# CloudEngineHub/MARL-LLM

Measured on AMD Instinct MI355X. Metric: agent-steps/sec, higher is better.
Workload: dtype f64 (state, every index / flag / reward decision) + f32 (obs, prior, action I/O, pre-filters); 1 GPU; assembly env, 64 agents x 4096 envs per GPU (64 x 4096 total), assembled state, prior-policy actions; agents=64, envs_per_gpu=4096, envs_total=4096, obs_dtype=f32, state_dtype=f64, seed=226, parallelism=env-sharded x1, no collective on the step path

## Files before the change

### marl_llm_amd/csrc/swarm_env.hip

```cpp

#include <hip/hip_runtime.h>

#include <algorithm>
#include <cmath>
#include <cstdint>
#include <cstdio>
#include <cstring>
#include <mutex>
#include <new>
#include <string>
#include <type_traits>
#include <utility>
#include <vector>

#include "swarm_env.h"
#include "swarm_internal.h"

namespace {

constexpr int kTopoMax = 6;
constexpr int kNeiStride = 8;
typedef unsigned long long u64;

struct LatEnv {
    double ox, oy;
    double uxi, uyi, vxi, vyi;
    float R, Rc;
    int nrows, ncols;
    short rowstart[64];
    unsigned long long rowmask[64];
};

struct KP {
    int n_env, n_a, ng_max, ngw, topo, g_max, occ_max, obs_dim;
    int with_self, periodic, boundary, with_prior, export_idx;
    int export_small;
    int cxy_stride;
    int cxq_stride;
    int g_stride;
    int off_cxy, off_sp, off_cmask, off_sbits, off_obits, off_sidx, off_snei, off_sncf, off_snear, off_pc;
    int smem_lat, smem_lat_export, smem_generic;
    double c_sen, c_near, c_occ, c_avoid, c_ball;
    double c_close, c_close2;
    float csen_lo, csen_hi, cocc_lo, cocc_hi;
    float coord_lim;
    float min_tol_a, min_tol_b;
    float rew_ga, rew_gb;
    int force_exact;
    int cap_int;
    unsigned cap_magic; int cap_shift;
    int cap_even;
    int dbg_phase, dbg_extra;
    int off_cxyf, off_partc, off_lat, off_cov, off_flag;
    int off_hdr, off_srow, off_pcr, off_perm, off_rres, off_orow, off_partd;
    float rew_ga_lat, rew_gb_lat;
    float rew_thr_k;
    int lattice;
    int lat_rw, lat_cw;
    int lat_nrs, lat_nrc;
    int lat_n32;
    double c_near_hi;
    const LatEnv *lat;
    double d_sen, r_avoid, size_a, size2, k_ball, k_wall, c_wall, vel_max, dt;
    double bx0, by1, bx2, by3, w_half, h_half;
    double *p, *dp;
    int *nei, *near_cell, *in_flag;
    double2 *sf_next;
    const double *cells;
    const double2 *cells_xy;
    const int *n_g;
    const double *c_in;
    int *exp_sensed, *exp_occ;
    void *prior_next;
    double pk_att, pk_rep, pk_ali;
    double pk_llm;
    int llm;
    double2 *act_next;
    long long *stamps;
};

typedef float f2v __attribute__((ext_vector_type(2)));

template <typename T> struct Pair;
template <> struct Pair<float>  { typedef float2 type; };
template <> struct Pair<double> { typedef double2 type; };
typedef __attribute__((ext_vector_type(2))) __bf16 bf2v;
template <> struct Pair<__bf16> { typedef bf2v type; };

template <typename OT> __device__ __forceinline__ OT to_out(double v) { return (OT)v; }
typedef double d2v __attribute__((ext_vector_type(2)));
__device__ __forceinline__ void store_nt(float2 *dst, float2 v) { f2v t = {v.x, v.y}; __builtin_nontemporal_store(t, reinterpret_cast<f2v *>(dst)); }
__device__ __forceinline__ void store_nt(double2 *dst, double2 v) { d2v t = {v.x, v.y}; __builtin_nontemporal_store(t, reinterpret_cast<d2v *>(dst)); }
__device__ __forceinline__ void store_nt(bf2v *dst, bf2v v) { __builtin_nontemporal_store(v, dst); }
template <> __device__ __forceinline__ __bf16 to_out<__bf16>(double v) { return (__bf16)(float)v; }

__device__ __forceinline__ void wrap_rel(double &x, double &y, double wh, double hh)
{
    if (x < -wh) x += 2 * wh; else if (x > wh) x -= 2 * wh;
    if (y < -hh) y += 2 * hh; else if (y > hh) y -= 2 * hh;
}


template <int LANE>
__device__ __forceinline__ int writelane_c(int value, int old)
{
    asm("s_nop 1\n\tv_writelane_b32 %0, %1, %2" : "+v"(old) : "s"(value), "n"(LANE));
    return old;
}

__device__ __forceinline__ unsigned shl1_or_mask(unsigned acc, unsigned long long mask)
{
    unsigned long long carry_out;
    asm("s_nop 1\n\tv_addc_co_u32_e64 %0, %1, %2, %2, %3" : "=v"(acc), "=s"(carry_out) : "v"(acc), "s"(mask));
    return acc;
}

__device__ __forceinline__ void pair_tests5(double d2u, double d2, double c_nb, double c_hi, double c_ht, double c_cd, double c_c1,
                                            unsigned &nb, unsigned &hi, unsigned &ht, unsigned &cd, unsigned &c1)
{
    unsigned long long m0, m1, m2, m3, m4;
    asm("v_cmp_lt_f64_e64 %5, %10, %12\n\t"
        "v_cmp_lt_f64_e64 %6, %10, %13\n\t"
        "v_cmp_lt_f64_e64 %7, %10, %14\n\t"
        "v_cmp_lt_f64_e64 %8, %11, %15\n\t"
        "v_cmp_lt_f64_e64 %9, %11, %16\n\t"
        "v_addc_co_u32_e64 %0, %5, %0, %0, %5\n\t"
        "v_addc_co_u32_e64 %1, %6, %1, %1, %6\n\t"
        "v_addc_co_u32_e64 %2, %7, %2, %2, %7\n\t"
        "v_addc_co_u32_e64 %3, %8, %3, %3, %8\n\t"
        "v_addc_co_u32_e64 %4, %9, %4, %4, %9"
        : "+v"(nb), "+v"(hi), "+v"(ht), "+v"(cd), "+v"(c1), "=&s"(m0), "=&s"(m1), "=&s"(m2), "=&s"(m3), "=&s"(m4)
        : "v"(d2u), "v"(d2), "s"(c_nb), "s"(c_hi), "s"(c_ht), "s"(c_cd), "s"(c_c1));
}

__device__ __forceinline__ void pair_tests6(double d2u, double d2, double c_nb, double c_hi, double c_ht, double c_cd, double c_c1, double c_c2,
                                            unsigned &nb, unsigned &hi, unsigned &ht, unsigned &cd, unsigned &c1, unsigned &c2)
{
    unsigned long long m0, m1, m2, m3, m4, m5;
    asm("v_cmp_lt_f64_e64 %6, %12, %14\n\t"
        "v_cmp_lt_f64_e64 %7, %12, %15\n\t"
        "v_cmp_lt_f64_e64 %8, %12, %16\n\t"
        "v_cmp_lt_f64_e64 %9, %13, %17\n\t"
        "v_cmp_lt_f64_e64 %10, %13, %18\n\t"
        "v_cmp_lt_f64_e64 %11, %13, %19\n\t"
        "v_addc_co_u32_e64 %0, %6, %0, %0, %6\n\t"
        "v_addc_co_u32_e64 %1, %7, %1, %1, %7\n\t"
        "v_addc_co_u32_e64 %2, %8, %2, %2, %8\n\t"
        "v_addc_co_u32_e64 %3, %9, %3, %3, %9\n\t"
        "v_addc_co_u32_e64 %4, %10, %4, %4, %10\n\t"
        "v_addc_co_u32_e64 %5, %11, %5, %5, %11"
        : "+v"(nb), "+v"(hi), "+v"(ht), "+v"(cd), "+v"(c1), "+v"(c2), "=&s"(m0), "=&s"(m1), "=&s"(m2), "=&s"(m3), "=&s"(m4), "=&s"(m5)
        : "v"(d2u), "v"(d2), "s"(c_nb), "s"(c_hi), "s"(c_ht), "s"(c_cd), "s"(c_c1), "s"(c_c2));
}

template <typename F, int... I>
__device__ __forceinline__ void static_for_impl(F &&f, std::integer_sequence<int, I...>)
{
    (f(std::integral_constant<int, I>{}), ...);
}
template <int N, typename F>
__device__ __forceinline__ void static_for(F &&f)
{
    static_for_impl(static_cast<F &&>(f), std::make_integer_sequence<int, N>{});
}

__device__ __forceinline__ double clamp_ref(double v, double lo, double hi)
{
    double m = (hi < v) ? hi : v;
    return (lo < m) ? m : lo;
}

#define REPS(k) ((P.dbg_phase == (k)) ? P.dbg_extra + 1 : 1)
#define FENCE() asm volatile("" ::: "memory")
#define EXIT_AT(k) do { if (P.dbg_phase == 15 && P.dbg_extra == (k)) return; } while (0)

#ifdef SWARM_STAMPS
#define STAMP(k) do { __builtin_amdgcn_sched_barrier(0); if (P.stamps != nullptr && (threadIdx.x & 63) == 0) P.stamps[((size_t)blockIdx.x * (blockDim.x >> 6) + (threadIdx.x >> 6)) * 24 + (k)] = clock64(); __builtin_amdgcn_sched_barrier(0); } while (0)
#else
#define STAMP(k) do { } while (0)
#endif

template <int NPAD, bool HALF = false> struct Geo {
    static_assert(!HALF || NPAD < 64, "the half-occupied geometry is for N < 64");
    static constexpr int NPAD_ = NPAD; static constexpr bool HALF_ = HALF;
    static constexpr bool CT_MAP = NPAD >= 64 || HALF;
    static constexpr int AG = NPAD < 64 ? 64 : NPAD;
    static constexpr int EPB = NPAD < 64 ? (64 / NPAD) / (HALF ? 2 : 1) : 1;
    static constexpr int ACTW = NPAD < 64 ? EPB * NPAD : 64;
    static constexpr int LPA = HALF ? 8 : 4;
    static constexpr int AGW = 64 / LPA;
    static constexpr int NW = AG / 64;
    static constexpr int WPE = 4;
    static constexpr int T = AG * WPE;
#ifndef SWARM_WPS
#define SWARM_WPS 7
#endif
#ifndef SWARM_WPS_SMALL
#define SWARM_WPS_SMALL 6
#endif
#ifndef SWARM_WPS_128
#define SWARM_WPS_128 6
#endif
    static constexpr int WPS_LAT = NPAD == 64 ? SWARM_WPS : (NPAD < 64 ? SWARM_WPS_SMALL : (NPAD == 128 ? SWARM_WPS_128 : 1));
    static constexpr int WPS_GEN = NPAD == 64 ? 6 : (NPAD < 64 ? 5 : 1);
};

template <int NPAD, bool HALF> struct LatMap {
    typedef Geo<NPAD, HALF> G_;
    static constexpr int AG = G_::AG, EPB = G_::EPB, NW = G_::NW, WPE = G_::WPE, T = G_::T;
    static constexpr int NRC = 16;
    static constexpr int al(int bytes) { return (bytes + 15) & ~15; }
    static constexpr int mx(int a, int b) { return a > b ? a : b; }
    static constexpr int sp_bytes = 4 * AG * 8;
    static constexpr int hdr_bytes = AG * 16;
    static constexpr int rew_scratch_bytes = NW * 1536;
    static constexpr int srow_bytes = mx((NRC - 1) * AG * 4, rew_scratch_bytes);
    static constexpr int pcr_bytes = AG * NRC;
    static constexpr int partc_bytes = WPE * AG * 2;
    static constexpr int partd_bytes = (WPE - 1) * AG * 8;
    static constexpr int lat_bytes = EPB * 64 * (8 + 2);
    static constexpr int cov_bytes = EPB * 64 * 8;
    static constexpr int flag_bytes = AG;
    static constexpr int snei_bytes = AG * kNeiStride * 2;
    static constexpr int sncf_bytes = AG * 4;
    static constexpr int snear_bytes = NW > 1 ? NW * AG * 8 : 0;
    static constexpr int orow_bytes = NRC * AG * 4;
    static constexpr int pm_bytes = (NW == 1 ? WPE * 4 : 5) * NW * AG * 8;
    static constexpr int sp = 0;
    static constexpr int hdr = sp + al(sp_bytes);
    static constexpr int srow = hdr + al(hdr_bytes);
    static constexpr int pcr = srow + al(srow_bytes);
    static constexpr int partc = pcr + al(pcr_bytes);
    static constexpr int partd = partc + al(partc_bytes);
    static constexpr int lat = partd + al(partd_bytes);
    static constexpr int cov = lat + al(lat_bytes);
    static constexpr int flag = cov + al(cov_bytes);
    static constexpr int snei = flag + al(flag_bytes);
    static constexpr int sncf = snei + al(snei_bytes);
    static constexpr int snear = sncf + al(sncf_bytes);
    static constexpr int sidx = snear + al(snear_bytes);
    static constexpr int perm = partd;
    static constexpr int perm_bytes = T, prk_bytes = WPE * AG * 2;
    static constexpr int sidx_bytes(int g_stride) { return al(mx(AG * g_stride * 2, pm_bytes)); }
    static constexpr int total(int g_stride) { return sidx + sidx_bytes(g_stride); }
    static constexpr int orow_off(int g_stride) { return total(g_stride); }
    static constexpr int total_export(int g_stride) { return orow_off(g_stride) + al(orow_bytes); }
    static_assert(perm_bytes <= partd_bytes, "perm must fit the distance array it reuses");
    static_assert(prk_bytes <= partc_bytes, "the partial ranks must fit the nearest-cell candidates they reuse");
    static_assert(rew_scratch_bytes <= srow_bytes, "the exact reward's scratch must fit the window rows it reuses");
    static_assert(pm_bytes <= sidx_bytes(0), "the pair masks must fit the list region they reuse");
};

constexpr double kSentinel = 1.0e200;

__device__ __forceinline__ double cospi01(double t)
{
    const bool flip = t > 0.5;
    const double r = flip ? 1.0 - t : t;
    const double x = M_PI * r;
    const double u = x * x;
    double c = -8.8967913924505741e-22;
    c = fma(c, u, 4.1103176233121648e-19);
    c = fma(c, u, -1.5619206968586225e-16);
    c = fma(c, u, 4.7794773323873853e-14);
    c = fma(c, u, -1.1470745597729725e-11);
    c = fma(c, u, 2.0876756987868100e-09);
    c = fma(c, u, -2.7557319223985888e-07);
    c = fma(c, u, 2.4801587301587302e-05);
    c = fma(c, u, -1.3888888888888889e-03);
    c = fma(c, u, 4.1666666666666664e-02);
    c = fma(c, u, -0.5);
    c = fma(c, u, 1.0);
    return flip ? -c : c;
}

__device__ __forceinline__ float psi_u_f32(float u)
{
    float c = 7.969553699e-04f;
    c = fmaf(c, u, -1.267949212e-02f);
    c = fmaf(c, u, 1.175149009e-01f);
    c = fmaf(c, u, -6.675792336e-01f);
    c = fmaf(c, u, 2.029347420e+00f);
    c = fmaf(c, u, -2.467400551e+00f);
    c = fmaf(c, u, 1.0f);
    return c;
}

__device__ __forceinline__ float psi5_u_f32(float u)
{
    float c = -1.028585434e-02f;
    c = fmaf(c, u, 1.148182452e-01f);
    c = fmaf(c, u, -6.661784649e-01f);
    c = fmaf(c, u, 2.029018402e+00f);
    c = fmaf(c, u, -2.467372179e+00f);
    c = fmaf(c, u, 9.999995828e-01f);
    return c;
}

template <int NPAD, typename OT, bool DO_STEP, bool LAT, bool HALF = false>
__global__ void __launch_bounds__((Geo<NPAD, HALF>::T), (LAT ? Geo<NPAD, HALF>::WPS_LAT : Geo<NPAD, HALF>::WPS_GEN))
k_env(const KP P, const void *__restrict__ action, const int act_f64, OT *__restrict__ obs,
      float *__restrict__ reward, uint8_t *__restrict__ done, OT *__restrict__ a_prior)
{
    typedef Geo<NPAD, HALF> G_;
    constexpr int AG = G_::AG, EPB = G_::EPB, NW = G_::NW, WPE = G_::WPE, T = G_::T;
    constexpr int ACTW = G_::ACTW, LPA = G_::LPA, AGW = G_::AGW;
    static_assert(!HALF || LAT, "the half-occupied geometry exists for the lattice path only");
    typedef typename Pair<OT>::type OT2;

    extern __shared__ __align__(16) unsigned char smem[];
    typedef LatMap<NPAD, HALF> LM;
#define LO(r) ((LAT && G_::CT_MAP) ? LM::r : P.off_##r)
    float *cxq = reinterpret_cast<float *>(smem + P.off_cxyf);
    double *sp = reinterpret_cast<double *>(smem + LO(sp));
    u64 *cmask = reinterpret_cast<u64 *>(smem + P.off_cmask);
    float *rsum = reinterpret_cast<float *>(smem + P.off_cmask);
    unsigned *sbits = reinterpret_cast<unsigned *>(smem + P.off_sbits);
    unsigned *obits = reinterpret_cast<unsigned *>(smem + P.off_obits);
    short *sidx = reinterpret_cast<short *>(smem + LO(sidx));
    typedef std::conditional_t<LAT, short, int> pc_t;
    pc_t *part_c = reinterpret_cast<pc_t *>(smem + LO(partc));
    u64 *pm = reinterpret_cast<u64 *>(smem + LO(sidx));
    unsigned *owords = reinterpret_cast<unsigned *>(smem + P.off_cmask);
    short *snei = reinterpret_cast<short *>(smem + LO(snei));
    int *sncf = reinterpret_cast<int *>(smem + LO(sncf));
    u64 *snear = reinterpret_cast<u64 *>(smem + LO(snear));
    u64 *lrm = reinterpret_cast<u64 *>(smem + LO(lat));
    short *lrs = reinterpret_cast<short *>(smem + LO(lat) + (size_t)EPB * 64 * 8);
    unsigned *cov = reinterpret_cast<unsigned *>(smem + LO(cov));
    int *sflag = reinterpret_cast<int *>(smem + LO(flag));
    unsigned char *pc = smem + P.off_pc;
    constexpr int NRC = LM::NRC;
    float4 *hdr = reinterpret_cast<float4 *>(smem + LO(hdr));
    unsigned *srow = reinterpret_cast<unsigned *>(smem + LO(srow));
    unsigned char *pcr = smem + LO(pcr);
    u64 *covrow = reinterpret_cast<u64 *>(smem + LO(cov));
    unsigned char *perm = smem + LO(perm);
    unsigned *orow = reinterpret_cast<unsigned *>(smem + P.off_orow);

    const int tid = threadIdx.x, lane = tid & 63;
    STAMP(0);
    const int at = tid % AG;
    const int sx = __builtin_amdgcn_readfirstlane((tid / AG + (int)blockIdx.x) % WPE);
    const int aw = at >> 6;
    auto flag_get = [&]() -> bool { return LAT ? ((reinterpret_cast<const unsigned *>(sflag)[at >> 2] >> ((at & 3) * 8)) & 1u) != 0 : (sflag[at] & 1) != 0; };
    const bool thr_on = NPAD >= 64 || at < ACTW;
    const int el = (NPAD < 64 && thr_on) ? at / NPAD : 0;
    const int i = NPAD < 64 ? at % NPAD : at;
    const int e = blockIdx.x * EPB + el;
    const int n_a = P.n_a;
    const bool act = thr_on && (e < P.n_env) && (i < n_a);
    const int es = e < P.n_env ? e : P.n_env - 1;
    const int ng = P.n_g[es];
    int ngb = ng;
    if (EPB > 1) {
        for (int k = 0; k < EPB; ++k) {
            const int ek = blockIdx.x * EPB + k;
            const int v = P.n_g[ek < P.n_env ? ek : P.n_env - 1];
            ngb = v > ngb ? v : ngb;
        }
    }
    const int W = (ngb + 31) >> 5;
    constexpr int SB = WPE > 1 ? 1 : 0;
    int w0 = W;
    if (WPE > 1) { w0 = (W - 2 * (WPE - 1)) / WPE; w0 = w0 < 0 ? 0 : w0; }
    auto mine = [&](int w) -> bool {
        if (WPE == 1) return true;
        if (w < w0) return sx == SB;
        const int o = (w - w0) % (WPE - 1);
        return sx == (o < SB ? o : o + 1);
    };
    const double2 *gce = P.cells_xy + (size_t)es * P.ng_max;
    auto cell64 = [&](int c) -> double2 { double2 g = gce[c < ng ? c : 0]; if (!(c < ng)) { g.x = kSentinel; g.y = kSentinel; } return g; };
    const float *cq_e = cxq + (size_t)el * P.cxq_stride;

    const size_t sbase = (size_t)es * 2 * n_a;
    double px = __builtin_nan(""), py = __builtin_nan(""), vx = 0.0, vy = 0.0;
    double ax = 0.0, ay = 0.0;
    double sf0x = 0.0, sf0y = 0.0;
    OT2 pri_now; pri_now.x = to_out<OT>(0.0); pri_now.y = to_out<OT>(0.0);
    const bool copy_prior = DO_STEP && P.with_prior && a_prior != nullptr;
    if (sx == 0 && act) {
        if (DO_STEP) { const double2 sfl = P.sf_next[(size_t)e * n_a + i]; sf0x = sfl.x; sf0y = sfl.y; }
        px = P.p[sbase + i]; py = P.p[sbase + n_a + i];
        vx = P.dp[sbase + i]; vy = P.dp[sbase + n_a + i];
        if (DO_STEP) {
            if (act_f64 & 2) {
                const size_t a0 = (size_t)e * n_a + i, a1 = a0 + (size_t)P.n_env * n_a;
                if (act_f64 & 1) { ax = ((const double *)action)[a0]; ay = ((const double *)action)[a1]; }
                else { ax = (double)((const float *)action)[a0]; ay = (double)((const float *)action)[a1]; }
            }
            else if (act_f64 & 1) { const size_t ab = ((size_t)e * n_a + i) * 2; ax = ((const double *)action)[ab]; ay = ((const double *)action)[ab + 1]; }
            else { const float2 af = reinterpret_cast<const float2 *>(action)[(size_t)e * n_a + i]; ax = (double)af.x; ay = (double)af.y; }
            if (copy_prior) pri_now = reinterpret_cast<const OT2 *>(P.prior_next)[(size_t)e * n_a + i];
        }
    }
    constexpr bool use_lat = LAT;
    if constexpr (!use_lat)
    for (int rep = 0, reps = REPS(9); rep < reps; ++rep)
    for (int k = 0; k < EPB; ++k) {
        FENCE();
        const int ek0 = blockIdx.x * EPB + k;
        const int ek = ek0 < P.n_env ? ek0 : P.n_env - 1;
        const int ngk = P.n_g[ek];
        const double *gx = P.cells + (size_t)ek * 2 * P.ng_max;
        const double *gy = gx + P.ng_max;
        for (int c = tid; c < W * 32; c += T) {
            double2 g;
            g.x = c < ngk ? gx[c] : kSentinel;
            g.y = c < ngk ? gy[c] : kSentinel;
            float *q = cxq + (size_t)k * P.cxq_stride + (c >> 1) * 4 + (c & 1);
            q[0] = (float)g.x; q[2] = (float)g.y;
        }
    }
    if (sx == 0) { if constexpr (LAT) { if ((at & 3) == 0) sflag[at >> 2] = 0; } else sflag[at] = 0; }
    if constexpr (use_lat) {
        for (int q = tid; q < EPB * 64; q += T) {
            const int ek0 = blockIdx.x * EPB + (q >> 6);
            const LatEnv &Lq = P.lat[ek0 < P.n_env ? ek0 : P.n_env - 1];
            lrm[q] = Lq.rowmask[q & 63]; lrs[q] = Lq.rowstart[q & 63];
            covrow[q] = 0;
        }
        if (sx == WPE - 1) reinterpret_cast<uint4 *>(pcr)[at] = uint4{0u, 0u, 0u, 0u};
    }
    double npx = px, npy = py, nvx = vx, nvy = vy;
    auto forces_integrate = [&]() {
        for (int rep = 0, reps = REPS(1); rep < reps; ++rep) {
            FENCE();
            const double sfx = sf0x, sfy = sf0y;
            STAMP(8);
            double Fx = 1 * ax + sfx, Fy = 1 * ay + sfy;
            if (P.boundary) {
                const double d0 = px - P.size_a - P.bx0;
                const double d1 = P.by1 - (py + P.size_a);
                const double d2 = P.bx2 - (px + P.size_a);
                const double d3 = py - P.size_a - P.by3;
                const double a0 = d0 < 0 ? fabs(d0) : 0.0, a1 = d1 < 0 ? fabs(d1) : 0.0;
                const double a2 = d2 < 0 ? fabs(d2) : 0.0, a3 = d3 < 0 ? fabs(d3) : 0.0;
                const double sx_ = (a0 - a2) * P.k_wall, sy_ = (a3 - a1) * P.k_wall;
                const double v0 = d0 < 0 ? vx : 0.0, v2 = d2 < 0 ? vx : 0.0;
                const double v3 = d3 < 0 ? vy : 0.0, v1 = d1 < 0 ? vy : 0.0;
                const double gx = (-v0 - v2) * P.c_wall, gy = (-v3 - v1) * P.c_wall;
                Fx = Fx + sx_ + gx;
                Fy = Fy + sy_ + gy;
            }
            STAMP(10);
            nvx = vx + (Fx / 1.0) * P.dt; nvy = vy + (Fy / 1.0) * P.dt;
            nvx = nvx < -P.vel_max ? -P.vel_max : (nvx > P.vel_max ? P.vel_max : nvx);
            nvy = nvy < -P.vel_max ? -P.vel_max : (nvy > P.vel_max ? P.vel_max : nvy);
            npx = px + nvx * P.dt; npy = py + nvy * P.dt;
            if (P.periodic) {
                if (npx < P.bx0) npx += 2 * P.w_half;
                if (npx > P.bx2) npx -= 2 * P.w_half;
                if (npy < P.by3) npy += 2 * P.h_half;
                if (npy > P.by1) npy -= 2 * P.h_half;
            }
        }
    };
    auto publish_new_state = [&]() {
        sp[at] = npx; sp[AG + at] = npy; sp[2 * AG + at] = nvx; sp[3 * AG + at] = nvy;
        if (DO_STEP && act) {
            P.p[sbase + i] = npx; P.p[sbase + n_a + i] = npy;
            P.dp[sbase + i] = nvx; P.dp[sbase + n_a + i] = nvy;
            if (copy_prior) store_nt(&reinterpret_cast<OT2 *>(a_prior)[(size_t)e * n_a + i], pri_now);
        }
    };
    if (sx == 0) {
        STAMP(11);
        __builtin_amdgcn_s_setprio(3);
        if (DO_STEP) forces_integrate();
        publish_new_state();
        __builtin_amdgcn_s_setprio(0);
        STAMP(12);
    }
    __syncthreads();
    STAMP(1);
    EXIT_AT(0);
    px = sp[at]; py = sp[AG + at];
    STAMP(2);
    EXIT_AT(1);

    constexpr int JN = NPAD < 64 ? NPAD : 64;
    const double *spx = sp + el * NPAD, *spy = sp + AG + el * NPAD;
    u64 nearbyN[NW], candN[NW], cand1N[NW], cand2N[NW], hitN[NW] = {};
    constexpr int CS = SB;
    {
        constexpr int JQ = JN / WPE;
        static_assert(JQ * WPE == JN && JQ <= 32, "pair pass: JN must split evenly into <= 32 agents per split");
        constexpr int PMK = 4;
        unsigned a_nb[1], a_cd[1], a_c1[1], a_ht[1];
        bool exc = false;
        auto place = [&](unsigned acc) -> u64 { return (u64)(__brev(acc) >> (32 - JQ)) << (sx * JQ); };
        for (int rep = 0, reps = REPS(2); rep < reps; ++rep) {
            FENCE();
            exc = false;
#pragma unroll 1
            for (int w = 0; w < NW; ++w) {
                unsigned nb = 0, cd = 0, c1 = 0, ht = 0, c2 = 0, a_hi = 0;
                const double *qx = spx + w * 64 + sx * JQ, *qy = spy + w * 64 + sx * JQ;
                auto pairs = [&](auto per_c) {
                    const bool PER = per_c;
                    static_assert(JQ % 2 == 0, "pair pass: two agents per LDS read");
#pragma unroll
                    for (int q = 0; q < JQ; q += 2) {
                        const double2 x2 = *reinterpret_cast<const double2 *>(qx + q), y2 = *reinterpret_cast<const double2 *>(qy + q);
#pragma unroll
                        for (int h = 0; h < 2; ++h) {
                            double rx = (h ? x2.y : x2.x) - px, ry = (h ? y2.y : y2.x) - py;
                            const double d2u = rx * rx + ry * ry;
                            double d2 = d2u;
                            if (PER) { wrap_rel(rx, ry, P.w_half, P.h_half); d2 = rx * rx + ry * ry; }
                            if constexpr (NW > 2)
                                pair_tests6(d2u, d2, P.c_near, P.c_near_hi, P.c_ball, P.c_sen, P.c_close, P.c_close2, nb, a_hi, ht, cd, c1, c2);
                            else
                                pair_tests5(d2u, d2, P.c_near, P.c_near_hi, P.c_ball, P.c_sen, P.c_close, nb, a_hi, ht, cd, c1);
                        }
                    }
                };
                if constexpr (LAT) { if (P.periodic) pairs(std::true_type{}); else pairs(std::false_type{}); }
                else pairs(P.periodic != 0);
                exc = exc || (a_hi != nb);
                if constexpr (NPAD < 64) { a_nb[0] = nb; a_cd[0] = cd; a_c1[0] = c1; a_ht[0] = ht; }
                else if (rep == reps - 1) {
                    unsigned short *pq = reinterpret_cast<unsigned short *>(pm) + sx;
                    auto quarter = [](unsigned acc) -> unsigned short { return (unsigned short)(__brev(acc) >> 16); };
                    pq[((size_t)(0 * NW + w) * AG + at) * 4] = quarter(nb);
                    pq[((size_t)(1 * NW + w) * AG + at) * 4] = quarter(cd);
                    pq[((size_t)(2 * NW + w) * AG + at) * 4] = quarter(c1);
                    pq[((size_t)(3 * NW + w) * AG + at) * 4] = quarter(ht);
                    if constexpr (NW > 2) pq[((size_t)(4 * NW + w) * AG + at) * 4] = quarter(c2);
                }
            }
        }
        STAMP(14);
        if (use_lat && exc) atomicOr(reinterpret_cast<unsigned *>(sflag) + (at >> 2), 1u << ((at & 3) * 8));
        if constexpr (NPAD < 64) {
#pragma unroll
            for (int w = 0; w < NW; ++w) {
                const u64 nbm = place(a_nb[w]);
                pm[((sx * PMK + 0) * NW + w) * AG + at] = NPAD < 64 ? (nbm << (el * NPAD)) : nbm;
                pm[((sx * PMK + 1) * NW + w) * AG + at] = place(a_cd[w]);
                pm[((sx * PMK + 2) * NW + w) * AG + at] = place(a_c1[w]);
                pm[((sx * PMK + 3) * NW + w) * AG + at] = place(a_ht[w]);
            }
            __syncthreads();
            nearbyN[0] = 0; candN[0] = 0; cand1N[0] = 0; cand2N[0] = 0;
#pragma unroll
            for (int q = 0; q < WPE; ++q) nearbyN[0] |= pm[(q * PMK + 0) * AG + at];
            if (sx == SB) {
#pragma unroll
                for (int q = 0; q < WPE; ++q) { candN[0] |= pm[(q * PMK + 1) * AG + at]; cand1N[0] |= pm[(q * PMK + 2) * AG + at]; }
            }
            if (sx == SB) {
#pragma unroll
                for (int q = 0; q < WPE; ++q) hitN[0] |= pm[(q * PMK + 3) * AG + at];
                hitN[0] &= ~(1ull << i);
            }
        } else {
            __syncthreads();
#pragma unroll
            for (int w = 0; w < NW; ++w) {
                nearbyN[w] = pm[(0 * NW + w) * AG + at]; candN[w] = 0; cand1N[w] = 0; cand2N[w] = 0;
                if (sx == SB) { candN[w] = pm[(1 * NW + w) * AG + at]; cand1N[w] = pm[(2 * NW + w) * AG + at]; cand2N[w] = pm[(4 * NW + w) * AG + at]; }
            }
            if (sx == CS) {
#pragma unroll
                for (int w = 0; w < NW; ++w) {
                    hitN[w] = pm[(3 * NW + w) * AG + at];
                    if (w == (i >> 6)) hitN[w] &= ~(1ull << (i & 63));
                }
            }
        }
    }
    const u64 nearby1 = nearbyN[0];
    STAMP(15);
    EXIT_AT(2);
    if (NW > 1 && sx == SB) __builtin_amdgcn_s_setprio(2);
    if (sx == SB) for (int rep = 0, reps = REPS(10); rep < reps; ++rep) {
        FENCE();
        bool collision = false;
        double nd[kTopoMax]; int nj[kTopoMax];
#pragma unroll
        for (int k = 0; k < kTopoMax; ++k) { nd[k] = INFINITY; nj[k] = -1; }
        u64 nearby[NW], cand[NW];
        {
            u64 c1[NW]; int n1 = 0;
#pragma unroll
            for (int w = 0; w < NW; ++w) { nearby[w] = nearbyN[w]; cand[w] = candN[w]; c1[w] = cand1N[w]; }
            if (i < 64 * NW) { const u64 self = ~(1ull << (i & 63)); cand[NPAD <= 64 ? 0 : (i >> 6)] &= self; c1[NPAD <= 64 ? 0 : (i >> 6)] &= self; }
#pragma unroll
            for (int w = 0; w < NW; ++w) n1 += __popcll(c1[w]);
            const bool few = n1 >= P.topo;
            if constexpr (NW > 2) {
                u64 c2[NW]; int n2 = 0;
#pragma unroll
                for (int w = 0; w < NW; ++w) c2[w] = cand2N[w];
                if (i < 64 * NW) c2[i >> 6] &= ~(1ull << (i & 63));
#pragma unroll
                for (int w = 0; w < NW; ++w) n2 += __popcll(c2[w]);
                const bool some = n2 >= P.topo;
#pragma unroll
                for (int w = 0; w < NW; ++w) cand[w] = some ? c2[w] : cand[w];
            }
#pragma unroll
            for (int w = 0; w < NW; ++w) cand[w] = few ? c1[w] : cand[w];
        }
        double dmin = INFINITY;
        {
            double nk[kTopoMax + 1];
#pragma unroll
            for (int k = 0; k <= kTopoMax; ++k) nk[k] = INFINITY;
#pragma unroll
            for (int w = 0; w < NW; ++w) {
                u64 h = cand[w];
                while (h) {
                    const int jj = __ffsll((unsigned long long)h) - 1;
                    h &= h - 1;
                    double rx = spx[w * 64 + jj] - px, ry = spy[w * 64 + jj] - py;
                    if (P.periodic) wrap_rel(rx, ry, P.w_half, P.h_half);
                    const double cd = rx * rx + ry * ry;
                    dmin = fmin(dmin, cd);
                    double key = __builtin_bit_cast(double, (__builtin_bit_cast(u64, cd) & ~0xFFull) | (u64)(w * 64 + jj));
#pragma unroll
                    for (int k = 0; k <= kTopoMax; ++k) {
                        const double lo = fmin(nk[k], key);
                        key = fmax(nk[k], key);
                        nk[k] = lo;
                    }
                }
            }
            bool amb = false;
#pragma unroll
            for (int k = 0; k < kTopoMax; ++k) {
                const u64 kb = __builtin_bit_cast(u64, nk[k]), kn = __builtin_bit_cast(u64, nk[k + 1]);
                const bool fin = nk[k] < INFINITY;
                nj[k] = fin ? (int)(kb & 0xFFull) : -1;
                amb = amb || (fin && nk[k + 1] < INFINITY && ((kb ^ kn) >> 8) == 0);
            }
            if (__any(amb)) {
                int xj[kTopoMax];
#pragma unroll
                for (int k = 0; k < kTopoMax; ++k) { nd[k] = INFINITY; xj[k] = -1; }
#pragma unroll
                for (int w = 0; w < NW; ++w) {
                    u64 h = amb ? cand[w] : 0;
                    while (h) {
                        const int jj = __ffsll((unsigned long long)h) - 1;
                        h &= h - 1;
                        double rx = spx[w * 64 + jj] - px, ry = spy[w * 64 + jj] - py;
                        if (P.periodic) wrap_rel(rx, ry, P.w_half, P.h_half);
                        double cd = sqrt(rx * rx + ry * ry); int cj = w * 64 + jj;
                        bool ins = false;
#pragma unroll
                        for (int k = 0; k < kTopoMax; ++k) {
                            const bool sw = ins || cd < nd[k];
                            ins = sw;
                            const double td = nd[k]; const int tjj = xj[k];
                            nd[k] = sw ? cd : td; xj[k] = sw ? cj : tjj;
                            cd = sw ? td : cd;    cj = sw ? tjj : cj;
                        }
                    }
                }
#pragma unroll
                for (int k = 0; k < kTopoMax; ++k) nj[k] = amb ? xj[k] : nj[k];
            }
        }
        STAMP(13);
        if constexpr (NW > 1) {
#pragma unroll
            for (int w = 0; w < NW; ++w) snear[w * AG + at] = nearby[w];
        }
#pragma unroll
        for (int k = 0; k < kTopoMax; ++k) {
            const bool used = k < P.topo && nj[k] >= 0;
            snei[at * kNeiStride + k] = (short)(used ? nj[k] : -1);
            if (P.export_small && act && k < P.topo) P.nei[((size_t)e * n_a + i) * P.topo + k] = used ? nj[k] : -1;
        }
        collision = dmin < P.c_avoid;
        snei[at * kNeiStride + kTopoMax] = (short)(collision ? 1 : 0);
    }
    if (sx == CS) {
        double sfx = 0.0, sfy = 0.0;
        for (int rep = 0, reps = REPS(1); rep < reps; ++rep) {
            FENCE();
            sfx = 0.0; sfy = 0.0;
#pragma unroll
            for (int w = 0; w < NW; ++w) {
                u64 h = hitN[w];
                while (h) {
                    const int kk = __ffsll((unsigned long long)h) - 1;
                    h &= h - 1;
                    const double dx = spx[w * 64 + kk] - px, dy = spy[w * 64 + kk] - py;
                    const double dc = sqrt(dx * dx + dy * dy);
                    const double de = fabs(dc - P.size2);
                    double wx = dx, wy = dy;
                    if (P.periodic) wrap_rel(wx, wy, P.w_half, P.h_half);
                    const double ux = wx / dc, uy = wy / dc;
                    sfx += 1.0 * de * P.k_ball * (-ux);
                    sfy += 1.0 * de * P.k_ball * (-uy);
                }
            }
        }
        if (act) P.sf_next[(size_t)e * n_a + i] = make_double2(sfx, sfy);
        if (NW > 1) __builtin_amdgcn_s_setprio(0);
    }
    STAMP(3);
    EXIT_AT(3);

    const float pxf = (float)px, pyf = (float)py;
    const bool lane_far = act && !(fabs(px) <= (double)P.coord_lim && fabs(py) <= (double)P.coord_lim);
    const bool wave_exact = (P.force_exact != 0) || (__any(lane_far) != 0);
    float best32 = INFINITY, second32 = INFINITY; int bc = 0;
    const f2v pxx = {pxf, pxf}, pyy = {pyf, pyf};
    if constexpr (use_lat) {
        const LatEnv &L = P.lat[es];
        const double apd = (px - L.ox) * L.uxi + (py - L.oy) * L.uyi;
        const double bpd = (px - L.ox) * L.vxi + (py - L.oy) * L.vyi;
        const float apf = (float)apd, bpf = (float)bpd;
        const int nrows = L.nrows, ncols = L.ncols;
        const float lat_m = fmaxf(1e-4f, 8e-7f * fmaxf(fabsf(apf), fabsf(bpf)));
        const int b0s = (int)ceilf(bpf - (L.R + 2.0f * lat_m));
        int ca0 = (int)ceilf(apf - (L.R + 2.0f * lat_m));
        ca0 = ca0 < 0 ? 0 : (ca0 > 63 ? 63 : ca0);
        if (sx == 0) {
            float4 hq;
            hq.x = (float)(apd - (double)ca0); hq.y = (float)(bpd - (double)b0s);
            hq.z = __int_as_float(b0s); hq.w = __int_as_float(ca0);
            hdr[at] = hq;
        }
        const u64 *rm = lrm + el * 64;
        const short *rs = lrs + el * 64;
        constexpr int WS = WPE > 1 ? WPE - 1 : 1;
        const int wr = WPE > 1 ? (sx < SB ? sx : sx - 1) : 0;
        auto walk = [&](auto tag) {
        typedef decltype(tag) MT;
        constexpr int MB = (int)sizeof(MT) * 8;
        auto rowmask = [&](int b) -> MT { return MB == 32 ? (MT)reinterpret_cast<const unsigned *>(rm)[2 * b] : (MT)rm[b]; };
        auto popc = [](MT v) -> int { return MB == 32 ? __popc((unsigned)v) : __popcll((unsigned long long)v); };
        auto ffs0 = [](MT v) -> int { return (MB == 32 ? __ffs((unsigned)v) : __ffsll((unsigned long long)v)) - 1; };
        auto range = [](int lo, int hi) -> MT { return hi >= lo ? (MT)((~(MT)0 >> (MB - 1 - hi)) & (~(MT)0 << lo)) : (MT)0; };
        auto row_sel = [&](int b, float rho, double cut) -> MT {
            const bool rowok = act && b >= 0 && b < nrows;
            const float dy = (float)b - bpf, dy2 = dy * dy;
            const float ro = rho + lat_m, ri = rho - lat_m, ri2 = ri > 0.0f ? ri * ri : 0.0f;
            const float ho2 = ro * ro - dy2;
            const bool any_o = rowok && ho2 > 0.0f;
            const float ho = __builtin_amdgcn_sqrtf(fmaxf(ho2, 0.0f));
            int ao0 = (int)ceilf(apf - ho), ao1 = (int)floorf(apf + ho);
            ao0 = ao0 < 0 ? 0 : ao0; ao1 = ao1 > ncols - 1 ? ncols - 1 : ao1;
            const int bq = b < 0 ? 0 : (b > 63 ? 63 : b);
            const MT rowm = any_o ? rowmask(bq) : (MT)0;
            const int rst = rs[bq];
            const float e0 = (float)ao0 - apf, e1 = (float)ao1 - apf;
            const bool c0 = fmaf(e0, e0, dy2) < ri2, c1 = fmaf(e1, e1, dy2) < ri2;
            MT acc = range(ao0, ao1);
            MT bnd = (MT)((c0 ? (MT)0 : (MT)1 << (ao0 & (MB - 1))) | (c1 ? (MT)0 : (MT)1 << (ao1 & (MB - 1)))) & acc & rowm;
            acc &= ~bnd;
            while (__any(bnd != 0)) {
                if (bnd != 0) {
                    const int a = ffs0(bnd);
                    bnd &= bnd - 1;
                    const int c = rst + popc(rowm & (MT)(((MT)1 << a) - 1));
                    const double2 g = cell64(c);
                    const double ex = g.x - px, ey = g.y - py;
                    if (ex * ex + ey * ey < cut) acc |= (MT)1 << a;
                }
            }
            return rowm & acc;
        };
        for (int rep = 0, reps = REPS(3); rep < reps; ++rep) {
            FENCE();
            for (int t = wr; t < P.lat_nrs; t += WS)
                srow[t * AG + at] = (unsigned)(row_sel(b0s + t, L.R, P.c_sen) >> ca0);
            const int b0c = (int)ceilf(bpf - (L.Rc + 2.0f * lat_m));
            for (int t = wr; t < P.lat_nrc; t += WS) {
                const MT selc = row_sel(b0c + t, L.Rc, P.c_occ);
                const int bq = b0c + t < 0 ? 0 : (b0c + t > 63 ? 63 : b0c + t);
                if (selc != 0) {
                    if constexpr (MB == 32) atomicOr(reinterpret_cast<unsigned *>(&covrow[el * 64 + bq]), (unsigned)selc);
                    else atomicOr(reinterpret_cast<unsigned long long *>(&covrow[el * 64 + bq]), (unsigned long long)selc);
                }
            }
            best32 = INFINITY; second32 = INFINITY; bc = 0;
            const int ar0 = (int)floorf(apf) + 1;
            const int a_r = ar0 < 0 ? 0 : (ar0 > MB - 1 ? MB - 1 : ar0);
            const MT lowm = (MT)(((MT)1 << a_r) - 1);
            const int nr_hi = EPB == 1 ? nrows : 64;
            auto row_cands = [&](int b, float &d2d, float &d2u, int &c_dn) {
                const MT rowm = (EPB == 1 || b < nrows) ? rowmask(b) : (MT)0;
// ... 2289 lines not shown
```

Baseline: 3.156 billion agent-steps/s.

## Exploit pair symmetry with a circulant split of the 64-agent pair pass

For 64-agent groups, the all-pairs distance tests now visit each pair once using circulant offsets: each split handles 8 offsets and scatters the compare results as forward and backward ballot masks. Positions are stored twice as interleaved double2 rows so the wrapped index reads are contiguous. The per-offset masks are rotated and OR-gathered after a barrier, roughly halving the distance and compare work. The cost is extra rotate, add-with-carry and shared-memory traffic, plus reliance on inline asm and fiddly bit-shift packing that could contain correctness risk.

```diff
diff --git a/marl_llm_amd/csrc/swarm_env.hip b/marl_llm_amd/csrc/swarm_env.hip
--- a/marl_llm_amd/csrc/swarm_env.hip
+++ b/marl_llm_amd/csrc/swarm_env.hip
@@ -153,6 +153,40 @@
         : "v"(d2u), "v"(d2), "s"(c_nb), "s"(c_hi), "s"(c_ht), "s"(c_cd), "s"(c_c1), "s"(c_c2));
 }
 
+__device__ __forceinline__ void pair_cmp5(double d2u, double d2, double c_nb, double c_hi, double c_ht, double c_cd, double c_c1,
+                                          unsigned long long &m0, unsigned long long &m1, unsigned long long &m2,
+                                          unsigned long long &m3, unsigned long long &m4)
+{
+    asm("v_cmp_lt_f64_e64 %0, %5, %7\n\t"
+        "v_cmp_lt_f64_e64 %1, %5, %8\n\t"
+        "v_cmp_lt_f64_e64 %2, %5, %9\n\t"
+        "v_cmp_lt_f64_e64 %3, %6, %10\n\t"
+        "v_cmp_lt_f64_e64 %4, %6, %11"
+        : "=&s"(m0), "=&s"(m1), "=&s"(m2), "=&s"(m3), "=&s"(m4)
+        : "v"(d2u), "v"(d2), "s"(c_nb), "s"(c_hi), "s"(c_ht), "s"(c_cd), "s"(c_c1));
+}
+
+__device__ __forceinline__ void pair_acc10(unsigned &f0, unsigned &f1, unsigned &f2, unsigned &f3, unsigned &f4,
+                                           unsigned &b0, unsigned &b1, unsigned &b2, unsigned &b3, unsigned &b4,
+                                           unsigned long long m0, unsigned long long m1, unsigned long long m2,
+                                           unsigned long long m3, unsigned long long m4,
+                                           unsigned long long r0, unsigned long long r1, unsigned long long r2,
+                                           unsigned long long r3, unsigned long long r4)
+{
+    asm("v_addc_co_u32_e64 %0, %10, %0, %0, %10\n\t"
+        "v_addc_co_u32_e64 %1, %11, %1, %1, %11\n\t"
+        "v_addc_co_u32_e64 %2, %12, %2, %2, %12\n\t"
+        "v_addc_co_u32_e64 %3, %13, %3, %3, %13\n\t"
+        "v_addc_co_u32_e64 %4, %14, %4, %4, %14\n\t"
+        "v_addc_co_u32_e64 %5, %15, %5, %5, %15\n\t"
+        "v_addc_co_u32_e64 %6, %16, %6, %6, %16\n\t"
+        "v_addc_co_u32_e64 %7, %17, %7, %7, %17\n\t"
+        "v_addc_co_u32_e64 %8, %18, %8, %8, %18\n\t"
+        "v_addc_co_u32_e64 %9, %19, %9, %9, %19"
+        : "+v"(f0), "+v"(f1), "+v"(f2), "+v"(f3), "+v"(f4), "+v"(b0), "+v"(b1), "+v"(b2), "+v"(b3), "+v"(b4),
+          "+s"(m0), "+s"(m1), "+s"(m2), "+s"(m3), "+s"(m4), "+s"(r0), "+s"(r1), "+s"(r2), "+s"(r3), "+s"(r4));
+}
+
 template <typename F, int... I>
 __device__ __forceinline__ void static_for_impl(F &&f, std::integer_sequence<int, I...>)
 {
@@ -203,6 +237,10 @@
 #endif
     static constexpr int WPS_LAT = NPAD == 64 ? SWARM_WPS : (NPAD < 64 ? SWARM_WPS_SMALL : (NPAD == 128 ? SWARM_WPS_128 : 1));
     static constexpr int WPS_GEN = NPAD == 64 ? 6 : (NPAD < 64 ? 5 : 1);
+#ifndef SWARM_PAIR_CIRC
+#define SWARM_PAIR_CIRC 1
+#endif
+    static constexpr bool CIRC = SWARM_PAIR_CIRC && NPAD == 64;
 };
 
 template <int NPAD, bool HALF> struct LatMap {
@@ -241,6 +279,8 @@
     static constexpr int sidx = snear + al(snear_bytes);
     static constexpr int perm = partd;
     static constexpr int perm_bytes = T, prk_bytes = WPE * AG * 2;
+    static constexpr int pdup = srow;
+    static constexpr int pdup_bytes = G_::CIRC ? 2 * 2 * AG * 8 : 0;
     static constexpr int sidx_bytes(int g_stride) { return al(mx(AG * g_stride * 2, pm_bytes)); }
     static constexpr int total(int g_stride) { return sidx + sidx_bytes(g_stride); }
     static constexpr int orow_off(int g_stride) { return total(g_stride); }
@@ -249,6 +289,7 @@
     static_assert(prk_bytes <= partc_bytes, "the partial ranks must fit the nearest-cell candidates they reuse");
     static_assert(rew_scratch_bytes <= srow_bytes, "the exact reward's scratch must fit the window rows it reuses");
     static_assert(pm_bytes <= sidx_bytes(0), "the pair masks must fit the list region they reuse");
+    static_assert(pdup_bytes <= srow_bytes, "the doubled position rows must fit the window rows they precede");
 };
 
 constexpr double kSentinel = 1.0e200;
@@ -305,6 +346,7 @@
     typedef Geo<NPAD, HALF> G_;
     constexpr int AG = G_::AG, EPB = G_::EPB, NW = G_::NW, WPE = G_::WPE, T = G_::T;
     constexpr int ACTW = G_::ACTW, LPA = G_::LPA, AGW = G_::AGW;
+    constexpr bool CIRC = LAT && G_::CIRC;
     static_assert(!HALF || LAT, "the half-occupied geometry exists for the lattice path only");
     typedef typename Pair<OT>::type OT2;
 
@@ -459,6 +501,10 @@
     };
     auto publish_new_state = [&]() {
         sp[at] = npx; sp[AG + at] = npy; sp[2 * AG + at] = nvx; sp[3 * AG + at] = nvy;
+        if constexpr (CIRC) {
+            double2 *pd = reinterpret_cast<double2 *>(smem + LM::pdup);
+            pd[at] = pd[AG + at] = make_double2(npx, npy);
+        }
         if (DO_STEP && act) {
             P.p[sbase + i] = npx; P.p[sbase + n_a + i] = npy;
             P.dp[sbase + i] = nvx; P.dp[sbase + n_a + i] = nvy;
@@ -484,7 +530,68 @@
     const double *spx = sp + el * NPAD, *spy = sp + AG + el * NPAD;
     u64 nearbyN[NW], candN[NW], cand1N[NW], cand2N[NW], hitN[NW] = {};
     constexpr int CS = SB;
-    {
+    if constexpr (CIRC) {
+        static_assert(NW == 1 && EPB == 1 && WPE == 4, "circulant pair pass: one 64-agent group, four splits");
+        constexpr int PMK = 4;
+        unsigned f_nb = 0, f_hi = 0, f_ht = 0, f_cd = 0, f_c1 = 0, b_nb = 0, b_hi = 0, b_ht = 0, b_cd = 0, b_c1 = 0;
+        const int k0 = sx * 8;
+        const double2 *dxy = reinterpret_cast<const double2 *>(smem + LM::pdup) + at + k0;
+        for (int rep = 0, reps = REPS(2); rep < reps; ++rep) {
+            FENCE();
+            f_nb = f_hi = f_ht = f_cd = f_c1 = b_nb = b_hi = b_ht = b_cd = b_c1 = 0;
+            auto pairs = [&](auto per_c) {
+                constexpr bool PER = decltype(per_c)::value;
+                auto dist = [&](int q, double &d2u, double &d2) {
+                    const double2 pj = dxy[q];
+                    double rx = pj.x - px, ry = pj.y - py;
+                    d2u = rx * rx + ry * ry;
+                    d2 = d2u;
+                    if (PER) { wrap_rel(rx, ry, P.w_half, P.h_half); d2 = rx * rx + ry * ry; }
+                };
+                double d2u, d2;
+                if (sx == 0) {
+                    dist(0, d2u, d2);
+                    pair_tests5(d2u, d2, P.c_near, P.c_near_hi, P.c_ball, P.c_sen, P.c_close, f_nb, f_hi, f_ht, f_cd, f_c1);
+                }
+                auto both = [&](int q) {
+                    dist(q, d2u, d2);
+                    u64 m0, m1, m2, m3, m4;
+                    pair_cmp5(d2u, d2, P.c_near, P.c_near_hi, P.c_ball, P.c_sen, P.c_close, m0, m1, m2, m3, m4);
+                    const int k = k0 + q;
+                    auto rot = [&](u64 m) -> u64 { return (m << k) | (m >> (64 - k)); };
+                    pair_acc10(f_nb, f_hi, f_ht, f_cd, f_c1, b_nb, b_hi, b_ht, b_cd, b_c1, m0, m1, m2, m3, m4,
+                               rot(m0), rot(m1), rot(m2), rot(m3), rot(m4));
+                };
+#pragma unroll
+                for (int q = 1; q < 8; ++q) both(q);
+                if (sx == WPE - 1) {
+                    dist(8, d2u, d2);
+                    pair_tests5(d2u, d2, P.c_near, P.c_near_hi, P.c_ball, P.c_sen, P.c_close, b_nb, b_hi, b_ht, b_cd, b_c1);
+                }
+                else both(8);
+            };
+            if (P.periodic) pairs(std::true_type{}); else pairs(std::false_type{});
+        }
+        STAMP(14);
+        if ((f_hi != f_nb) || (b_hi != b_nb)) atomicOr(reinterpret_cast<unsigned *>(sflag) + (at >> 2), 1u << ((at & 3) * 8));
+        const int shf = sx == WPE - 1 ? 0 : 23 - k0, shb = 24 - k0;
+        auto word = [&](unsigned f, unsigned b) -> u64 { return (u64)(__brev(f) >> shf) | ((u64)(b << shb) << 32); };
+        pm[(0 * WPE + sx) * AG + at] = word(f_nb, b_nb);
+        pm[(1 * WPE + sx) * AG + at] = word(f_cd, b_cd);
+        pm[(2 * WPE + sx) * AG + at] = word(f_c1, b_c1);
+        pm[(3 * WPE + sx) * AG + at] = word(f_ht, b_ht);
+        static_assert(PMK * WPE * AG * 8 <= LM::pm_bytes, "the partial words must fit the pair-mask region");
+        __syncthreads();
+        auto gather = [&](int m) -> u64 {
+            u64 o = 0;
+#pragma unroll
+            for (int q = 0; q < WPE; ++q) o |= pm[(m * WPE + q) * AG + at];
+            return (o << at) | (o >> ((64 - at) & 63));
+        };
+        nearbyN[0] = gather(0); candN[0] = 0; cand1N[0] = 0; cand2N[0] = 0;
+        if (sx == SB) { candN[0] = gather(1); cand1N[0] = gather(2); }
+        if (sx == CS) hitN[0] = gather(3) & ~(1ull << i);
+    } else {
         constexpr int JQ = JN / WPE;
         static_assert(JQ * WPE == JN && JQ <= 32, "pair pass: JN must split evenly into <= 32 agents per split");
         constexpr int PMK = 4;
```

New measurement: 3.112 billion agent-steps/s. 0.986x the previous value.
